# RobotLocomotion/pytorch-dense-correspondence

Hardware: AMD Instinct MI355X
Metric: training images/sec, 640x480 D=3 ResNet34-8s (higher is better)
Workload: dtype f32 (f16x3 products)

## Files before the change

pytorch-dense-correspondence_amd/csrc/conv_kernels.hip:

```cpp
#include "conv_shared.h"
#include "dcn_tuning.h"

namespace {

using namespace dcnconv;

template <int WM, int TM, int TN, int BK, bool TR>
__device__ __forceinline__ void gemm_segment(const GemmConv& p, float* lds, int tile, int k0, int k1, int nk, float* slot) {
    using G = GemmGeo<WM, TM, TN, BK>;
    constexpr int BM = G::BM, BN = G::BN, LDK = G::LDK, KQ = G::KQ, ROWS = G::ROWS, PA = G::PA, PB = G::PB,
                  kStage = G::kStage;
    const int tid = threadIdx.x, lane = tid & 63, wv = tid >> 6;
    const int wm_ = WM == 2 ? (wv >> 1) : 0, wn_ = WM == 2 ? (wv & 1) : wv;
    const int mt = fdiv(tile, p.div_nt), nt = tile - mt * p.ntiles;
    const int m0 = mt * BM, n0 = nt * BN;

    const int kq = tid % KQ, r0 = tid / KQ;
    int by[PA], bx[PA], pixbase[PA];
#pragma unroll
    for (int j = 0; j < PA; ++j) {
        const int m = m0 + r0 + ROWS * j;
        const int mm = m < p.M ? m : 0;
        const int img = fdiv(mm, p.div_hw), rem = mm - img * p.div_hw.d;
        const int y = fdiv(rem, p.div_w), x = rem - y * p.div_w.d;
// ... 412 lines not shown
            store_tile(cur ^ 1);
            mfma_steps(0);
#pragma unroll
            for (int i = 0; i < 16; ++i) {
                __builtin_amdgcn_sched_group_barrier(0x008, 1, 0);
                __builtin_amdgcn_sched_group_barrier(0x306, 3, 0);
            }
            __syncthreads();
            load_tile(m_begin + (st + 2 < nsteps ? st + 2 : nsteps - 1) * WK);
            read_frags(cur ^ 1, 0, 0);
            mfma_steps(1);
#pragma unroll
            for (int i = 0; i < 16; ++i) {
                __builtin_amdgcn_sched_group_barrier(0x008, 1, 0);
                __builtin_amdgcn_sched_group_barrier(0x126, 6, 0);
            }
        }
    }
    float* out = p.slab + (int64_t)split * p.cout * p.K;
    const int kc = j0 + wn_ * 64 + 2 * fi;
    if (kc < p.K) {
#pragma unroll
        for (int tm = 0; tm < 2; ++tm) {
#pragma unroll
            for (int r = 0; r < 16; ++r) {
                const int n = n0 + wm_ * 64 + 2 * ((r & 3) + 8 * (r >> 2) + 4 * fh) + tm;
                if (n < p.cout)
                    *reinterpret_cast<float2*>(out + (int64_t)n * p.K + kc) = make_float2(acc[tm][0][r], acc[tm][1][r]);
            }
        }
    }
}

__global__ void __launch_bounds__(256)
wgrad_reduce_kernel(const float* __restrict__ slab, float* __restrict__ dw, int64_t n4, int splits) {
    const int64_t i = (int64_t)blockIdx.x * 256 + threadIdx.x;
    if (i >= n4) return;
    const float4* src = reinterpret_cast<const float4*>(slab) + i;
    float4 a = src[0];
    int s = 1;
    for (; s + 4 <= splits; s += 4) {
        const float4 b0 = src[(int64_t)s * n4], b1 = src[(int64_t)(s + 1) * n4], b2 = src[(int64_t)(s + 2) * n4],
                     b3 = src[(int64_t)(s + 3) * n4];
        a.x += b0.x; a.y += b0.y; a.z += b0.z; a.w += b0.w;
        a.x += b1.x; a.y += b1.y; a.z += b1.z; a.w += b1.w;
        a.x += b2.x; a.y += b2.y; a.z += b2.z; a.w += b2.w;
        a.x += b3.x; a.y += b3.y; a.z += b3.z; a.w += b3.w;
    }
    for (; s < splits; ++s) {
        const float4 b = src[(int64_t)s * n4];
        a.x += b.x; a.y += b.y; a.z += b.z; a.w += b.w;
    }
    reinterpret_cast<float4*>(dw)[i] = a;
}

__global__ void __launch_bounds__(256)
wgrad_reduce_wide_kernel(const float* __restrict__ slab, float* __restrict__ dw, int64_t n4, int splits) {
    __shared__ float4 part[16][16];
    const int c = threadIdx.x & 15, sl = threadIdx.x >> 4;
    const int64_t i = (int64_t)blockIdx.x * 16 + c;
    float4 a = make_float4(0.f, 0.f, 0.f, 0.f);
    if (i < n4) {
        const float4* src = reinterpret_cast<const float4*>(slab) + i;
        int s = sl;
        for (; s + 48 < splits; s += 64) {
            const float4 b0 = src[(int64_t)s * n4], b1 = src[(int64_t)(s + 16) * n4], b2 = src[(int64_t)(s + 32) * n4],
                         b3 = src[(int64_t)(s + 48) * n4];
            a.x += b0.x; a.y += b0.y; a.z += b0.z; a.w += b0.w;
            a.x += b1.x; a.y += b1.y; a.z += b1.z; a.w += b1.w;
            a.x += b2.x; a.y += b2.y; a.z += b2.z; a.w += b2.w;
            a.x += b3.x; a.y += b3.y; a.z += b3.z; a.w += b3.w;
        }
        for (; s < splits; s += 16) {
            const float4 b = src[(int64_t)s * n4];
            a.x += b.x; a.y += b.y; a.z += b.z; a.w += b.w;
        }
    }
    part[sl][c] = a;
    __syncthreads();
    if (sl == 0 && i < n4) {
#pragma unroll
        for (int k = 1; k < 16; ++k) {
            const float4 b = part[k][c];
            a.x += b.x; a.y += b.y; a.z += b.z; a.w += b.w;
        }
        reinterpret_cast<float4*>(dw)[i] = a;
    }
}

__global__ void __launch_bounds__(256)
transpose_weight_kernel(const float* __restrict__ w, float* __restrict__ wt, int cout, int taps, int cin, int ldn) {
    __shared__ float tile[32][33];
    const int tap = blockIdx.z;
    const int c0 = blockIdx.x * 32, n0 = blockIdx.y * 32;
    const int tx = threadIdx.x & 31, ty = threadIdx.x >> 5;
    for (int i = ty; i < 32; i += 8) {
        const int n = n0 + i, c = c0 + tx;
        tile[i][tx] = (n < cout && c < cin) ? w[((int64_t)n * taps + tap) * cin + c] : 0.f;
    }
    __syncthreads();
    for (int i = ty; i < 32; i += 8) {
        const int c = c0 + i, n = n0 + tx;
        if (c < cin && n < ldn) wt[((int64_t)c * taps + tap) * ldn + n] = tile[tx][i];
    }
}

int wgrad_splits(const dcn_conv_desc* c, int* rows_per_split) {
    const int M = c->n * c->hout * c->wout, K = c->kh * c->kw * c->cin;
    const bool narrow = c->cout <= 64;
    const int tiles = dcn::ceil_div(c->cout, narrow ? 64 : 128) * dcn::ceil_div(K, narrow ? 256 : 128);
    int splits = dcn::ceil_div(2048, tiles);
    const int max_by_rows = (M / (8 * WK)) > 1 ? (M / (8 * WK)) : 1;
    if (splits > max_by_rows) splits = max_by_rows;
    const int cap = narrow ? 256 : 64;
    if (splits > cap) splits = cap;
    if (splits < 1) splits = 1;
    int rps = dcn::ceil_div(dcn::ceil_div(M, splits), WK) * WK;
    splits = dcn::ceil_div(M, rps);
    *rows_per_split = rps;
    return splits;
}

bool valid_desc(const dcn_conv_desc* c) {
    return c && c->n > 0 && c->hin > 0 && c->win > 0 && c->cin > 0 && (c->cin % 4) == 0 && c->hout > 0 && c->wout > 0 &&
           c->cout > 0 && c->kh > 0 && c->kw > 0 && c->stride > 0 && c->dil > 0 && c->pad >= 0 && c->ldc >= c->cout;
}

}

namespace dcnconv {
void launch_wgrad_reduce(const float* slabs, float* dw, int64_t n4, int splits, hipStream_t st) {
    if (splits >= 32) {
        hipLaunchKernelGGL(wgrad_reduce_wide_kernel, dim3((unsigned)dcn::ceil_div64(n4, 16)), dim3(256), 0, st, slabs, dw, n4, splits);
        return;
    }
    hipLaunchKernelGGL(wgrad_reduce_kernel, dim3((unsigned)dcn::ceil_div64(n4, 256)), dim3(256), 0, st, slabs, dw, n4,
                       splits);
}
}

extern "C" int dcn_conv_num_mtiles(const dcn_conv_desc* c) {
    if (!valid_desc(c)) return DCN_E_INVALID;
    return gemm_shape(c->n * c->hout * c->wout, c->cout, c->kh * c->kw * c->cin, c->group_rows).mtiles;
}

extern "C" size_t dcn_conv_gemm_workspace(const dcn_conv_desc* c, int dgrad) {
    if (!valid_desc(c)) return 0;
    if (dgrad) return gemm_shape(c->n * c->hin * c->win, c->cin, c->kh * c->kw * c->ldc).ws_bytes;
    return gemm_shape(c->n * c->hout * c->wout, c->cout, c->kh * c->kw * c->cin, c->group_rows).ws_bytes;
}

extern "C" int dcn_conv_forward(const dcn_conv_desc* c, const float* in, const float* w, const float* bias, float* out,
                                float* bn_partial, void* workspace, void* stream) {
    if (!valid_desc(c) || !in || !w || !out) return DCN_E_INVALID;
    GemmConv p;
    p.src = in; p.wm = w; p.bias = bias; p.add = nullptr; p.dst = out; p.bn_partial = bn_partial; p.out_absmax = nullptr;
    p.hs = c->hin; p.ws = c->win; p.cs = c->cin; p.hd = c->hout; p.wd = c->wout; p.cd = c->cout;
    p.kh = c->kh; p.kw = c->kw; p.stride = c->stride; p.pad = c->pad; p.dil = c->dil; p.ldc = c->ldc;
    p.M = c->n * c->hout * c->wout; p.K = c->kh * c->kw * c->cin; p.transposed = 0; p.relu = 0;
    return launch_gemm(p, workspace, (hipStream_t)stream, c->group_rows);
}

extern "C" int dcn_conv_dgrad(const dcn_conv_desc* c, const float* dout, const float* wt, const float* add, float* din,
                              void* workspace, void* stream) {
    if (!valid_desc(c) || !dout || !wt || !din || (c->ldc % 4) != 0) return DCN_E_INVALID;
    GemmConv p;
    p.src = dout; p.wm = wt; p.bias = nullptr; p.add = add; p.dst = din; p.bn_partial = nullptr; p.out_absmax = nullptr;
    p.hs = c->hout; p.ws = c->wout; p.cs = c->ldc;
    p.hd = c->hin; p.wd = c->win; p.cd = c->cin;
    p.kh = c->kh; p.kw = c->kw; p.stride = c->stride; p.pad = c->pad; p.dil = c->dil; p.ldc = c->cin;
// ... 42 lines not shown
```

pytorch-dense-correspondence_amd/csrc/conv_shared.h:

```cpp
#pragma once
#include <cstdlib>

#include "dcn_common.h"

namespace dcnconv {

typedef float f32x16 __attribute__((ext_vector_type(16)));

constexpr int NT = 256;

struct FastDiv {
    uint32_t mul, shr;
    int d;
};
inline FastDiv make_fastdiv(int d) {
    FastDiv f;
    f.d = d;
    uint32_t s = 0;
    while ((1u << s) < (uint32_t)d) ++s;
    f.shr = s;
    f.mul = (uint32_t)((((uint64_t)1 << 32) * (((uint64_t)1 << s) - (uint64_t)d)) / (uint64_t)d) + 1u;
    return f;
}
__device__ __forceinline__ int fdiv(int n, const FastDiv& f) { return (int)((__umulhi((uint32_t)n, f.mul) + (uint32_t)n) >> f.shr); }
// ... 220 lines not shown
            }
        }
    }
    if (p.bn_partial) {
#pragma unroll
        for (int tn = 0; tn < TN16; ++tn) {
            csum[tn] += __shfl_xor(csum[tn], 16, 64);
            csq[tn] += __shfl_xor(csq[tn], 16, 64);
            cmax[tn] = fmaxf(cmax[tn], __shfl_xor(cmax[tn], 16, 64));
            csum[tn] += __shfl_xor(csum[tn], 32, 64);
            csq[tn] += __shfl_xor(csq[tn], 32, 64);
            cmax[tn] = fmaxf(cmax[tn], __shfl_xor(cmax[tn], 32, 64));
            if (fq == 0) {
                const int cl = col0 + tn * 16 + fc;
                red[(wm * 3 + 0) * BN + cl] = csum[tn];
                red[(wm * 3 + 1) * BN + cl] = csq[tn];
                red[(wm * 3 + 2) * BN + cl] = cmax[tn];
            }
        }
        __syncthreads();
        if (tid < BN && n0 + tid < p.cd) {
            const float s = red[0 * BN + tid] + red[3 * BN + tid];
            const float q = red[1 * BN + tid] + red[4 * BN + tid];
            const float mx = fmaxf(red[2 * BN + tid], red[5 * BN + tid]);
            p.bn_partial[((int64_t)mt * 3 + 0) * p.cd + n0 + tid] = s;
            p.bn_partial[((int64_t)mt * 3 + 1) * p.cd + n0 + tid] = q;
            p.bn_partial[((int64_t)mt * 3 + 2) * p.cd + n0 + tid] = mx;
        }
    }
}

void launch_wgrad_reduce(const float* slabs, float* dw, int64_t n4, int splits, hipStream_t st);

}
```

pytorch-dense-correspondence_amd/csrc/dcn_tuning.h:

```cpp
#pragma once

namespace dcn {

struct Tuning {
    int conv_mode = -1;
    int conv_mode_invalid = 0;
    int backward_overlap = 1;
    int gemm_tile_m = 0;
    int gemm_sk = -1;
    double gemm_sk_min_gain = 20.0;
    int gemm_uni = 1;
    int stem8 = 1;
    int gemm_sk_inline = 1;
    int bn_bwd_fused = 0;
    int defer_residual_add = 1;
    int wgrad_splits = 0;
    int wgrad_tile = 0;
    int wgrad_deep = 4;
    int gemm_hl = 1;
    int hl_min_k = 128;
    int gemm_hl_rows = 0;
    int gemm_hlx = 1;
    int gemm_hlx_kg = 0;
    int gemm_hlx_splits = 0;
    int gemm_hlx_narrow = 1;
    double hlx_cost1 = 1.32, hlx_cost2 = 1.42, hlx_split_cost = 14.0;
    int hl_setprio = 1;
    int hlx_stagger = 1;
    int hlx_counters = 1;
    int wgrad_hl_min_m = 0;
    int wgrad_hl = 1;
    int wgrad_hlr = 1;
    int wgrad_hlr_min_m = 0;
    int wgrad_hlr_pairs = 1;
    int hl_producers = 1;
    int hl_only_mid = 1;
    int stem_pool_fused = 1;
    int bn_reduce_wide = 32;
    int wsplit_overlap = 1;
    int bn_nt = 0;
    int bn_reverse = 0;
    int wgrad_roles = 1;
};

const Tuning& tuning();

}
```

pytorch-dense-correspondence_amd/csrc/dcn_tuning.hip:

```cpp
#include <atomic>
#include <cstdio>
#include <cstdlib>
#include <cstring>
#include <mutex>

#include "dcn_common.h"
#include "dcn_tuning.h"

namespace dcn {
namespace {

Tuning g_tuning;
std::once_flag g_once;
std::mutex g_mu;

void read_env(Tuning& t) {
    t = Tuning();
    if (const char* m = getenv("DCN_CONV_MODE")) {
        if (!strcmp(m, "fp32")) t.conv_mode = DCN_CONV_FP32;
        else if (!strcmp(m, "f16x3")) t.conv_mode = DCN_CONV_F16X3;
        else t.conv_mode_invalid = 1;
    }
    if (const char* e = getenv("DCN_BACKWARD_OVERLAP")) t.backward_overlap = atoi(e) != 0;
    if (const char* e = getenv("DCN_GEMM_TILE_M")) t.gemm_tile_m = atoi(e);
// ... 8 lines not shown
    if (const char* e = getenv("DCN_WGRAD_ROLES")) t.wgrad_roles = atoi(e);
    if (const char* e = getenv("DCN_WGRAD_TILE")) t.wgrad_tile = atoi(e);
    if (const char* e = getenv("DCN_WGRAD_SPLITS")) t.wgrad_splits = atoi(e);
    if (const char* e = getenv("DCN_GEMM_HL")) t.gemm_hl = atoi(e);
    if (const char* e = getenv("DCN_GEMM_HL_ROWS")) t.gemm_hl_rows = atoi(e);
    if (const char* e = getenv("DCN_HL_MIN_K")) { const int v = atoi(e); if (v >= 32) t.hl_min_k = v; }
    if (const char* e = getenv("DCN_GEMM_HLX")) {
        int a = 0, b = 0;
        if (strchr(e, ',')) {
            if (sscanf(e, "%d,%d", &a, &b) == 2) {
                t.gemm_hlx = 1;
                t.gemm_hlx_kg = (a == 1 || a == 2) ? a : 0;
                t.gemm_hlx_splits = b > 0 ? b : 0;
            }
        } else {
            t.gemm_hlx = atoi(e) != 0;
        }
    }
    if (const char* e = getenv("DCN_GEMM_HLX_NARROW")) t.gemm_hlx_narrow = atoi(e) != 0;
    if (const char* e = getenv("DCN_HLX_COST")) {
        double a = 0, b = 0, c = 0;
        if (sscanf(e, "%lf,%lf,%lf", &a, &b, &c) == 3 && a > 0 && b > 0 && c >= 0) { t.hlx_cost1 = a; t.hlx_cost2 = b; t.hlx_split_cost = c; }
    }
    if (const char* e = getenv("DCN_HL_ONLY_MID")) t.hl_only_mid = atoi(e);
    if (const char* e = getenv("DCN_STEM_POOL_FUSED")) t.stem_pool_fused = atoi(e);
    if (const char* e = getenv("DCN_WGRAD_HL")) t.wgrad_hl = atoi(e);
    if (const char* e = getenv("DCN_HL_SETPRIO")) t.hl_setprio = atoi(e) != 0;
    if (const char* e = getenv("DCN_HLX_STAGGER")) { const int v = atoi(e); t.hlx_stagger = (v >= 0 && v <= 2) ? v : 1; }
    if (const char* e = getenv("DCN_HLX_COUNTERS")) t.hlx_counters = atoi(e) != 0;
    if (const char* e = getenv("DCN_WGRAD_HL_MIN_M")) t.wgrad_hl_min_m = atoi(e);
    if (const char* e = getenv("DCN_WGRAD_HLR")) t.wgrad_hlr = atoi(e);
    if (const char* e = getenv("DCN_WGRAD_HLR_MIN_M")) t.wgrad_hlr_min_m = atoi(e);
    if (const char* e = getenv("DCN_WGRAD_HLR_PAIRS")) t.wgrad_hlr_pairs = atoi(e);
    if (const char* e = getenv("DCN_HL_PRODUCERS")) t.hl_producers = atoi(e) != 0;
    if (const char* e = getenv("DCN_BN_REVERSE")) t.bn_reverse = atoi(e);
    if (const char* e = getenv("DCN_BN_NT")) t.bn_nt = atoi(e);
    if (const char* e = getenv("DCN_WSPLIT_OVERLAP")) t.wsplit_overlap = atoi(e) != 0;
    if (const char* e = getenv("DCN_BN_REDUCE_WIDE")) t.bn_reduce_wide = atoi(e);
}

}

const Tuning& tuning() {
    std::call_once(g_once, [] { read_env(g_tuning); });
    return g_tuning;
}

}

extern "C" void dcn_reload_env(void) {
    (void)dcn::tuning();
    std::lock_guard<std::mutex> lock(dcn::g_mu);
    dcn::read_env(dcn::g_tuning);
}
```

pytorch-dense-correspondence_amd/csrc/wgrad_hl_kernels.hip:

```cpp
#include <algorithm>
#include <type_traits>

#include "conv_shared.h"
#include "dcn_tuning.h"
#include "f16_split.h"

namespace {

using namespace dcnconv;
using namespace dcnsplit;

typedef __attribute__((address_space(3))) void* whl_lds_ptr;
typedef short s4v __attribute__((ext_vector_type(4)));

constexpr int kOob = (int)0x80000000;
constexpr int kStage = 65536;
constexpr int WPX = 32;

__device__ __forceinline__ void glds16(__amdgpu_buffer_rsrc_t rs, void* lds_dst, int voffset, int soffset) {
    __builtin_amdgcn_raw_ptr_buffer_load_lds(rs, (whl_lds_ptr)lds_dst, 16, voffset, soffset, 0, 0);
}
__device__ __forceinline__ s4v lds_tr4(const unsigned char* p) {
    return __builtin_amdgcn_ds_read_tr16_b64_v4i16((__attribute__((address_space(3))) s4v*)p);
}

struct WgradHl {
    const void* xh;
    const void* dh;
    float* slab;
    const float* x_absmax;
    const float* d_absmax;
    unsigned x_bytes, d_bytes;
    int hin, win, cin, cout, kh, kw, pad, dil, ldo, M, K, splits, stages_per_split, ntiles_n, ntiles_k, cpt, setprio;
    FastDiv div_hw, div_w, div_cpt, div_kw;
};

__global__ void __launch_bounds__(512, 1)
conv_wgrad_hl_kernel(WgradHl p) {
    __shared__ __attribute__((aligned(16))) unsigned char lds[2 * kStage];
    const int tid = threadIdx.x, lane = tid & 63;
    const int wv = __builtin_amdgcn_readfirstlane(tid >> 6);
    const int grp = wv >> 2, wn = wv & 3;
    const int tiles = p.ntiles_n * p.ntiles_k;
    const int bid = xcd_remap(blockIdx.x, tiles * p.splits);
    const int split = bid / tiles, tile = bid - split * tiles;
    const int tn_ = tile / p.ntiles_k, tk_ = tile - tn_ * p.ntiles_k;
    const int n0 = tn_ * 256, kc0 = tk_ * 256;
    const int nstages = (p.M + WPX - 1) / WPX;
    const int s_begin = split * p.stages_per_split;
    const int s_end = min(nstages, s_begin + p.stages_per_split);
    const int m_end = min(p.M, s_end * WPX);
    const __amdgpu_buffer_rsrc_t rs_x = __builtin_amdgcn_make_buffer_rsrc(const_cast<void*>(p.xh), 0, (int)p.x_bytes, 0x00020000);
    const __amdgpu_buffer_rsrc_t rs_d = __builtin_amdgcn_make_buffer_rsrc(const_cast<void*>(p.dh), 0, (int)p.d_bytes, 0x00020000);

    const int lp = lane >> 5, p16 = lane & 31;
    const int ldo4 = p.ldo * 4, cin4 = p.cin * 4;
    int kp[2];
    int cA[2][2], cB[2][2];
    int tdy[2][2], tdx[2][2];
#pragma unroll
    for (int e = 0; e < 2; ++e) {
        kp[e] = 4 * wv + 2 * e + lp;
        const int key = (kp[e] & 3) | (((kp[e] >> 3) & 1) << 2);
        const int unit = (p16 >> 1) ^ key;
        const int slot = unit >> 1;
        const int lc = slot >> 1, pl = slot & 1, q16 = 2 * (unit & 1) + (p16 & 1);
// ... 135 lines not shown
        else if (ph == 1) DCN_WAIT_VMCNT(0);
        DCN_WAIT_LGKMCNT0();
        bar();
        mfma_quadrant(qi, qj);
        bar();
    };
    using T = std::true_type;
    using F = std::false_type;
    if (s_begin < s_end) {
        issue_half(0, 0);
        issue_half(0, 1);
        issue_half(0, 2);
        issue_half(0, 3);
        advance();
        __builtin_amdgcn_sched_barrier(0);
        DCN_WAIT_VMCNT(4);
        bar();
        if (grp == 1) bar();
        int buf = 0;
        for (int s = s_begin; s + 1 < s_end; ++s) {
            phase(T{}, buf, 0);
            phase(T{}, buf, 1);
            phase(T{}, buf, 2);
            phase(T{}, buf, 3);
            buf ^= 1;
        }
        phase(F{}, buf, 0);
        phase(F{}, buf, 1);
        phase(F{}, buf, 2);
        phase(F{}, buf, 3);
        if (grp == 0) bar();
    }
    const float inv = 1.f / ((p.d_absmax ? pow2_scale(*p.d_absmax) : 1.f) * (p.x_absmax ? pow2_scale(*p.x_absmax) : 1.f));
    float* out = p.slab + (int64_t)split * p.cout * p.K;
    const int fc = lane & 15, fq4 = 4 * (lane >> 4);
#pragma unroll
    for (int tb = 0; tb < 8; ++tb)
#pragma unroll
        for (int cb = 0; cb < 4; ++cb) {
            const int kc = kc0 + wn * 64 + cb * 16 + fc;
#pragma unroll
            for (int r = 0; r < 4; ++r) {
                const int n = n0 + grp * 128 + tb * 16 + fq4 + r;
                if (n < p.cout && kc < p.K) out[(int64_t)n * p.K + kc] = acc[tb][cb][r] * inv;
            }
        }
}

bool wgrad_hl_supported(const dcn_conv_desc* c) {
    if (!c || c->n < 1 || c->hin < 1 || c->win < 32 || c->cin < 32 || c->cout < 32 || c->kh < 1 || c->kw < 1) return false;
    if (c->stride != 1 || c->hin != c->hout || c->win != c->wout || c->ldc != c->cout) return false;
    if ((c->cin % 32) != 0 || (c->cout % 32) != 0) return false;
    const int64_t xb = (int64_t)c->n * c->hin * c->win * c->cin * 4, db = (int64_t)c->n * c->hout * c->wout * c->ldc * 4;
    return xb <= ((int64_t)1 << 31) - 1 && db <= ((int64_t)1 << 31) - 1;
}

int wgrad_hl_splits(const dcn_conv_desc* c, int* stages_per_split) {
    const int M = c->n * c->hout * c->wout, K = c->kh * c->kw * c->cin;
    const int tiles = dcn::ceil_div(c->cout, 256) * dcn::ceil_div(K, 256);
    const int nstages = dcn::ceil_div(M, WPX);
    int best = 1;
    double best_score = -1.0;
    const int hi = std::min(nstages, std::max(1, 2 * 256 / tiles + 1));
    for (int s = 1; s <= hi; ++s) {
        const int sps = dcn::ceil_div(nstages, s), real = dcn::ceil_div(nstages, sps);
        const int wgs = real * tiles;
        const double eff = (double)wgs / (double)(dcn::ceil_div(wgs, 256) * 256);
        const double score = eff - 0.002 * real - (wgs < 256 ? 0.5 * (1.0 - wgs / 256.0) : 0.0) - (wgs > 256 ? 0.15 : 0.0);
        if (score > best_score) { best_score = score; best = s; }
    }
    if (const int v = dcn::tuning().wgrad_splits) { if (v >= 1 && v <= nstages) best = v; }
    const int sps = dcn::ceil_div(nstages, best);
    *stages_per_split = sps;
    return dcn::ceil_div(nstages, sps);
}


constexpr int RW_WP = 34;
constexpr int RW_DY_BYTES = 32 * 256;

template <int CB> struct RwGeom {
    static constexpr int kPitch = 256 * CB;
    static constexpr int kXInstr = (3 * RW_WP * kPitch + 8191) / 8192;
    static constexpr int kXBytes = kXInstr * 8192;
    static constexpr int kStageBytes = RW_DY_BYTES + kXBytes;
};

struct WgradHlr {
    const void* xh;
    const void* dh;
    float* slab;
    const float* x_absmax;
    const float* d_absmax;
    unsigned x_bytes, d_bytes;
    int hin, win, cin, cout, ldo, K, nstages, segs, splits, stages_per_split, ntiles_n, ntiles_c;
    FastDiv div_segs, div_h;
};

template <int CB>
__global__ void __launch_bounds__(512, 1)
conv_wgrad_hlr_kernel(WgradHlr p) {
    using G = RwGeom<CB>;
    constexpr int E = G::kXInstr, PITCH = G::kPitch;
    __shared__ __attribute__((aligned(16))) unsigned char lds[2 * G::kStageBytes];
    const int tid = threadIdx.x, lane = tid & 63;
    const int wv = __builtin_amdgcn_readfirstlane(tid >> 6);
    const int nh = wv & 1, cq = wv >> 1;
    const int tiles = p.ntiles_n * p.ntiles_c;
    const int bid = xcd_remap(blockIdx.x, tiles * p.splits);
    const int split = bid / tiles, tile = bid - split * tiles;
    const int tn_ = tile / p.ntiles_c, tc_ = tile - tn_ * p.ntiles_c;
    const int n0 = tn_ * 64, c0 = tc_ * 64 * CB;
    const int s_begin = split * p.stages_per_split;
    const int s_end = min(p.nstages, s_begin + p.stages_per_split);
    const __amdgpu_buffer_rsrc_t rs_x = __builtin_amdgcn_make_buffer_rsrc(const_cast<void*>(p.xh), 0, (int)p.x_bytes, 0x00020000);
    const __amdgpu_buffer_rsrc_t rs_d = __builtin_amdgcn_make_buffer_rsrc(const_cast<void*>(p.dh), 0, (int)p.d_bytes, 0x00020000);
    auto key_of = [](int pixel) { return (pixel & 3) | (((pixel >> 3) & 1) << 2); };

    auto unit_src = [](int u, int ps) { return (u >> 2) * 128 + ((u >> 1) & 1) * 64 + (u & 1) * 32 + (ps & 1) * 16; };
    const int dpix = 4 * wv + (lane >> 4);
    const int dsrc = (n0 / 32) * 128 + unit_src(((lane & 15) >> 1) ^ key_of(dpix), lane & 15);
    int xinfo[E];
#pragma unroll
    for (int e = 0; e < E; ++e) {
        const int byte = (wv + 8 * e) * 1024 + lane * 16;
        const int row = byte / PITCH, ps = (byte - row * PITCH) >> 4;
        const int r = row / RW_WP, q = row - r * RW_WP;
        xinfo[e] = unit_src((ps >> 1) ^ key_of(q), ps) | (q << 16) | ((row < 3 * RW_WP ? r + 1 : 0) << 24);
// ... 83 lines not shown
            if constexpr (CB == 1) DCN_WAIT_VMCNT(5); else DCN_WAIT_VMCNT(8);
        } else {
            __builtin_amdgcn_sched_barrier(0);
            DCN_WAIT_VMCNT(0);
        }
        __builtin_amdgcn_sched_barrier(0);
        __builtin_amdgcn_s_barrier();
        __builtin_amdgcn_sched_barrier(0);
        va = abase + buf * G::kStageBytes;
        DCN_OPAQUE_INT(va);
#pragma unroll
        for (int sft = 0; sft < 3; ++sft)
#pragma unroll
            for (int h = 0; h < 2; ++h) {
                vb[sft][h] = bbase[sft][h] + buf * G::kStageBytes;
                DCN_OPAQUE_INT(vb[sft][h]);
            }
        read_a();
#pragma unroll
        for (int tap = 0; tap < AH; ++tap) read_b(tap, tap);
#pragma unroll
        for (int tap = 0; tap < 9; ++tap) {
            if (tap + AH < 9) read_b(tap + AH, (tap + AH) % (AH + 1));
            __builtin_amdgcn_sched_barrier(0);
            mfma_tap(tap, tap % (AH + 1));
            __builtin_amdgcn_sched_barrier(0);
        }
        __builtin_amdgcn_sched_barrier(0);
        DCN_WAIT_LGKMCNT0();
        __builtin_amdgcn_s_barrier();
        __builtin_amdgcn_sched_barrier(0);
    }
    const float inv = 1.f / ((p.d_absmax ? pow2_scale(*p.d_absmax) : 1.f) * (p.x_absmax ? pow2_scale(*p.x_absmax) : 1.f));
    float* out = p.slab + (int64_t)split * p.cout * p.K;
    const int fc = lane & 15, fq4 = 4 * (lane >> 4);
#pragma unroll
    for (int i = 0; i < 2; ++i)
#pragma unroll
        for (int tap = 0; tap < 9; ++tap)
#pragma unroll
            for (int c = 0; c < CB; ++c) {
                const int kc = tap * p.cin + c0 + (CB * cq + c) * 16 + fc;
#pragma unroll
                for (int r = 0; r < 4; ++r) {
                    const int n = n0 + (2 * nh + i) * 16 + fq4 + r;
                    out[(int64_t)n * p.K + kc] = acc[i][tap][c][r] * inv;
                }
            }
}


constexpr int RP_DY_BYTES = 2 * 32 * 256;
constexpr int RP_XINSTR = 5;
constexpr int RP_STAGE = RP_DY_BYTES + RP_XINSTR * 8192;

__global__ void __launch_bounds__(512, 1)
conv_wgrad_hlrp_kernel(WgradHlr p) {
    constexpr int E = RP_XINSTR, PITCH = 256;
    __shared__ __attribute__((aligned(16))) unsigned char lds[2 * RP_STAGE];
    const int tid = threadIdx.x, lane = tid & 63;
    const int wv = __builtin_amdgcn_readfirstlane(tid >> 6);
    const int grp = wv >> 2, cq = wv & 3;
    const int tiles = p.ntiles_n * p.ntiles_c;
    const int bid = xcd_remap(blockIdx.x, tiles * p.splits);
    const int split = bid / tiles, tile = bid - split * tiles;
    const int tn_ = tile / p.ntiles_c, tc_ = tile - tn_ * p.ntiles_c;
// ... 118 lines not shown
        }
        __builtin_amdgcn_sched_barrier(0);
        DCN_WAIT_LGKMCNT0();
        __builtin_amdgcn_s_barrier();
        __builtin_amdgcn_sched_barrier(0);
    }
    float4* xch = reinterpret_cast<float4*>(lds);
#pragma unroll
    for (int half = 0; half < 2; ++half) {
        if (grp == 1) {
#pragma unroll
            for (int i = 0; i < 2; ++i)
#pragma unroll
                for (int tap = 0; tap < 9; ++tap) {
                    const f32x4_t v = acc[2 * half + i][tap];
                    xch[(cq * 18 + i * 9 + tap) * 64 + lane] = make_float4(v[0], v[1], v[2], v[3]);
                }
        }
        __syncthreads();
        if (grp == 0) {
#pragma unroll
            for (int i = 0; i < 2; ++i)
#pragma unroll
                for (int tap = 0; tap < 9; ++tap) {
                    const float4 v = xch[(cq * 18 + i * 9 + tap) * 64 + lane];
                    acc[2 * half + i][tap][0] += v.x; acc[2 * half + i][tap][1] += v.y;
                    acc[2 * half + i][tap][2] += v.z; acc[2 * half + i][tap][3] += v.w;
                }
        }
        __syncthreads();
    }
    if (grp != 0) return;
    const float inv = 1.f / ((p.d_absmax ? pow2_scale(*p.d_absmax) : 1.f) * (p.x_absmax ? pow2_scale(*p.x_absmax) : 1.f));
    float* out = p.slab + (int64_t)split * p.cout * p.K;
    const int fc = lane & 15, fq4 = 4 * (lane >> 4);
#pragma unroll
    for (int i = 0; i < 4; ++i)
#pragma unroll
        for (int tap = 0; tap < 9; ++tap) {
            const int kc = tap * p.cin + c0 + cq * 16 + fc;
#pragma unroll
            for (int r = 0; r < 4; ++r) out[(int64_t)(n0 + i * 16 + fq4 + r) * p.K + kc] = acc[i][tap][r] * inv;
        }
}

bool wgrad_hlr_supported(const dcn_conv_desc* c) {
    if (!c || c->n < 1 || c->hin < 1 || c->win < 1 || c->hout < 1 || c->wout < 1 || c->kh != 3 || c->kw != 3 || c->dil != 1 ||
        c->pad != 1) return false;
    if (c->stride != 1 || c->hin != c->hout || c->win != c->wout || c->ldc != c->cout) return false;
    if (c->cin < 64 || c->cout < 64 || (c->cin % 64) != 0 || (c->cout % 64) != 0) return false;
    const int64_t xb = (int64_t)c->n * c->hin * c->win * c->cin * 4, db = (int64_t)c->n * c->hout * c->wout * c->ldc * 4;
    return xb <= ((int64_t)1 << 31) - 1 && db <= ((int64_t)1 << 31) - 1;
}
bool hlr_pairs() { return dcn::tuning().wgrad_hlr_pairs != 0; }
int wgrad_hlr_stages(const dcn_conv_desc* c, bool pairs) {
    return c->n * (pairs ? dcn::ceil_div(c->hout, 2) : c->hout) * dcn::ceil_div(c->wout, 32);
}
int wgrad_hlr_splits(const dcn_conv_desc* c, int* stages_per_split, bool pairs) {
    const int nstages = wgrad_hlr_stages(c, pairs), tiles = (c->cout / 64) * (c->cin / 64);
    int s = std::max(1, std::min(std::max(256 / tiles, 1), nstages / 2));
    if (const int v = dcn::tuning().wgrad_splits) { if (v >= 1 && v <= nstages) s = v; }
    const int sps = dcn::ceil_div(nstages, s);
    *stages_per_split = sps;
    return dcn::ceil_div(nstages, sps);
}
bool use_hlr(const dcn_conv_desc* c) {
    const int v = dcn::tuning().wgrad_hlr;
    if (v == 0 || !wgrad_hlr_supported(c)) return false;
    if (v == 2) return true;
    if ((c->cout % 256) == 0) return false;
    if (dcn::tuning().wgrad_hlr_min_m > 0) return (int64_t)c->n * c->hout * c->wout >= dcn::tuning().wgrad_hlr_min_m;
    return (int64_t)c->n * c->hout * dcn::ceil_div(c->wout, 32) * (c->cout / 64) * (c->cin / 64) >= 2048;
}
int launch_wgrad_hlr(const dcn_conv_desc* c, const void* x_hl, const float* x_absmax, const void* dout_hl,
                     const float* dout_absmax, float* dw, void* slabs, hipStream_t st) {
    WgradHlr p;
    p.xh = x_hl; p.dh = dout_hl; p.x_absmax = x_absmax; p.d_absmax = dout_absmax;
    p.x_bytes = (unsigned)((int64_t)c->n * c->hin * c->win * c->cin * 4);
    p.d_bytes = (unsigned)((int64_t)c->n * c->hout * c->wout * c->ldc * 4);
    p.hin = c->hin; p.win = c->win; p.cin = c->cin; p.cout = c->cout; p.ldo = c->ldc; p.K = 9 * c->cin;
    p.segs = dcn::ceil_div(c->wout, 32); p.nstages = wgrad_hlr_stages(c, hlr_pairs());
    p.splits = wgrad_hlr_splits(c, &p.stages_per_split, hlr_pairs());
    p.ntiles_n = c->cout / 64; p.ntiles_c = c->cin / 64;
    p.div_segs = make_fastdiv(p.segs); p.div_h = make_fastdiv(hlr_pairs() ? dcn::ceil_div(c->hin, 2) : c->hin);
    p.slab = p.splits == 1 ? dw : (float*)slabs;
    if (hlr_pairs()) hipLaunchKernelGGL(conv_wgrad_hlrp_kernel, dim3(p.ntiles_n * p.ntiles_c * p.splits), dim3(512), 0, st, p);
    else hipLaunchKernelGGL(conv_wgrad_hlr_kernel<1>, dim3(p.ntiles_n * p.ntiles_c * p.splits), dim3(512), 0, st, p);
    if (p.splits > 1) launch_wgrad_reduce((const float*)slabs, dw, (int64_t)c->cout * p.K / 4, p.splits, st);
    return dcn::check_launch();
}
}

extern "C" int dcn_conv_wgrad_hl_eligible(const dcn_conv_desc* c) {
    if (dcn::tuning().wgrad_hl == 0) return 0;
    if (use_hlr(c)) return 1;
    if (!wgrad_hl_supported(c)) return 0;
    if (dcn::tuning().wgrad_hl == 2) return 1;
    const int64_t min_m = dcn::tuning().wgrad_hl_min_m > 0 ? dcn::tuning().wgrad_hl_min_m : 4096;
    return ((c->cout % 256) == 0 && c->kh * c->kw * c->cin >= std::min(1024, dcn::tuning().hl_min_k) &&
            (int64_t)c->n * c->hout * c->wout >= min_m) ? 1 : 0;
}

extern "C" int dcn_conv_wgrad_hl_kind(const dcn_conv_desc* c) { return use_hlr(c) ? 2 : (wgrad_hl_supported(c) ? 1 : 0); }

extern "C" size_t dcn_conv_wgrad_workspace_hl(const dcn_conv_desc* c) {
    size_t bytes = 0;
    int sps;
    if (wgrad_hlr_supported(c))
        bytes = (size_t)std::max(wgrad_hlr_splits(c, &sps, true), wgrad_hlr_splits(c, &sps, false)) * c->cout * 9 * c->cin * sizeof(float);
    if (wgrad_hl_supported(c))
        bytes = std::max(bytes, (size_t)wgrad_hl_splits(c, &sps) * c->cout * c->kh * c->kw * c->cin * sizeof(float));
    return bytes;
}

extern "C" int dcn_conv_wgrad_hl(const dcn_conv_desc* c, const void* x_hl, const float* x_absmax, const void* dout_hl,
                                 const float* dout_absmax, float* dw, void* slabs, void* stream) {
    if (!x_hl || !dout_hl || !dw || !slabs) return DCN_E_INVALID;
    if (use_hlr(c)) return launch_wgrad_hlr(c, x_hl, x_absmax, dout_hl, dout_absmax, dw, slabs, (hipStream_t)stream);
    if (!wgrad_hl_supported(c)) return DCN_E_UNSUPPORTED;
    WgradHl p;
    p.xh = x_hl; p.dh = dout_hl; p.x_absmax = x_absmax; p.d_absmax = dout_absmax;
    p.x_bytes = (unsigned)((int64_t)c->n * c->hin * c->win * c->cin * 4);
    p.d_bytes = (unsigned)((int64_t)c->n * c->hout * c->wout * c->ldc * 4);
    p.hin = c->hin; p.win = c->win; p.cin = c->cin; p.cout = c->cout; p.kh = c->kh; p.kw = c->kw; p.pad = c->pad; p.dil = c->dil;
    p.ldo = c->ldc; p.M = c->n * c->hout * c->wout; p.K = c->kh * c->kw * c->cin; p.cpt = c->cin / 32;
    p.splits = wgrad_hl_splits(c, &p.stages_per_split);
    p.setprio = dcn::tuning().hl_setprio;
    p.ntiles_n = dcn::ceil_div(c->cout, 256); p.ntiles_k = dcn::ceil_div(p.K, 256);
    p.div_hw = make_fastdiv(c->hout * c->wout); p.div_w = make_fastdiv(c->wout);
    p.div_cpt = make_fastdiv(p.cpt); p.div_kw = make_fastdiv(c->kw);
    p.slab = p.splits == 1 ? dw : (float*)slabs;
    hipStream_t st = (hipStream_t)stream;
    hipLaunchKernelGGL(conv_wgrad_hl_kernel, dim3(p.ntiles_n * p.ntiles_k * p.splits), dim3(512), 0, st, p);
    if (p.splits > 1) launch_wgrad_reduce((const float*)slabs, dw, (int64_t)c->cout * p.K / 4, p.splits, st);
    return dcn::check_launch();
}
```

Before: 465.4.

## Store split-K wgrad partials in fragment order and scatter during reduction

When weight-gradient GEMMs are split across multiple slabs, each wave now writes its accumulator fragments as contiguous float4 per lane in MFMA fragment order, instead of scattering them into the row-major dW layout. A new reduce kernel sums the slabs in that layout and maps each fragment back to its (cout, k) position when writing dW. This makes the partial-slab writes and reads fully coalesced, at the cost of strided scalar stores in the final reduce and extra index arithmetic. Workspace sizing for the non-HLR path is changed to cover whole padded tiles.

```diff
diff --git a/pytorch-dense-correspondence_amd/csrc/conv_kernels.hip b/pytorch-dense-correspondence_amd/csrc/conv_kernels.hip
--- a/pytorch-dense-correspondence_amd/csrc/conv_kernels.hip
+++ b/pytorch-dense-correspondence_amd/csrc/conv_kernels.hip
@@ -468,11 +468,7 @@
     }
 }
 
-__global__ void __launch_bounds__(256)
-wgrad_reduce_kernel(const float* __restrict__ slab, float* __restrict__ dw, int64_t n4, int splits) {
-    const int64_t i = (int64_t)blockIdx.x * 256 + threadIdx.x;
-    if (i >= n4) return;
-    const float4* src = reinterpret_cast<const float4*>(slab) + i;
+__device__ __forceinline__ float4 sum_slabs_in_order(const float4* __restrict__ src, int64_t n4, int splits) {
     float4 a = src[0];
     int s = 1;
     for (; s + 4 <= splits; s += 4) {
@@ -487,7 +483,31 @@
         const float4 b = src[(int64_t)s * n4];
         a.x += b.x; a.y += b.y; a.z += b.z; a.w += b.w;
     }
-    reinterpret_cast<float4*>(dw)[i] = a;
+    return a;
+}
+__device__ __forceinline__ float4 sum_slabs_of_lane(const float4* __restrict__ src, int64_t n4, int splits, int sl) {
+    float4 a = make_float4(0.f, 0.f, 0.f, 0.f);
+    int s = sl;
+    for (; s + 48 < splits; s += 64) {
+        const float4 b0 = src[(int64_t)s * n4], b1 = src[(int64_t)(s + 16) * n4], b2 = src[(int64_t)(s + 32) * n4],
+                     b3 = src[(int64_t)(s + 48) * n4];
+        a.x += b0.x; a.y += b0.y; a.z += b0.z; a.w += b0.w;
+        a.x += b1.x; a.y += b1.y; a.z += b1.z; a.w += b1.w;
+        a.x += b2.x; a.y += b2.y; a.z += b2.z; a.w += b2.w;
+        a.x += b3.x; a.y += b3.y; a.z += b3.z; a.w += b3.w;
+    }
+    for (; s < splits; s += 16) {
+        const float4 b = src[(int64_t)s * n4];
+        a.x += b.x; a.y += b.y; a.z += b.z; a.w += b.w;
+    }
+    return a;
+}
+
+__global__ void __launch_bounds__(256)
+wgrad_reduce_kernel(const float* __restrict__ slab, float* __restrict__ dw, int64_t n4, int splits) {
+    const int64_t i = (int64_t)blockIdx.x * 256 + threadIdx.x;
+    if (i >= n4) return;
+    reinterpret_cast<float4*>(dw)[i] = sum_slabs_in_order(reinterpret_cast<const float4*>(slab) + i, n4, splits);
 }
 
 __global__ void __launch_bounds__(256)
@@ -496,22 +516,7 @@
     const int c = threadIdx.x & 15, sl = threadIdx.x >> 4;
     const int64_t i = (int64_t)blockIdx.x * 16 + c;
     float4 a = make_float4(0.f, 0.f, 0.f, 0.f);
-    if (i < n4) {
-        const float4* src = reinterpret_cast<const float4*>(slab) + i;
-        int s = sl;
-        for (; s + 48 < splits; s += 64) {
-            const float4 b0 = src[(int64_t)s * n4], b1 = src[(int64_t)(s + 16) * n4], b2 = src[(int64_t)(s + 32) * n4],
-                         b3 = src[(int64_t)(s + 48) * n4];
-            a.x += b0.x; a.y += b0.y; a.z += b0.z; a.w += b0.w;
-            a.x += b1.x; a.y += b1.y; a.z += b1.z; a.w += b1.w;
-            a.x += b2.x; a.y += b2.y; a.z += b2.z; a.w += b2.w;
-            a.x += b3.x; a.y += b3.y; a.z += b3.z; a.w += b3.w;
-        }
-        for (; s < splits; s += 16) {
-            const float4 b = src[(int64_t)s * n4];
-            a.x += b.x; a.y += b.y; a.z += b.z; a.w += b.w;
-        }
-    }
+    if (i < n4) a = sum_slabs_of_lane(reinterpret_cast<const float4*>(slab) + i, n4, splits, sl);
     part[sl][c] = a;
     __syncthreads();
     if (sl == 0 && i < n4) {
@@ -521,6 +526,69 @@
             a.x += b.x; a.y += b.y; a.z += b.z; a.w += b.w;
         }
         reinterpret_cast<float4*>(dw)[i] = a;
+    }
+}
+
+template <int KIND>
+__device__ __forceinline__ void wgrad_frag_pos(int64_t q, const WgradFragMap& m, int& n, int& kc) {
+    constexpr int T4 = KIND == WGRAD_FRAG_TILE ? 256 * 256 / 4 : 64 * 576 / 4;
+    constexpr int FR = KIND == WGRAD_FRAG_TILE ? 32 : KIND == WGRAD_FRAG_ROWPAIR ? 36 : 18;
+    const int tile = (int)(q / T4), rem = (int)(q - (int64_t)tile * T4);
+    const int wv = rem / (FR * 64), f = (rem >> 6) - wv * FR, lane = rem & 63;
+    const int ta = tile / m.ntiles_minor, tb = tile - ta * m.ntiles_minor;
+    const int fc = lane & 15, fq4 = 4 * (lane >> 4);
+    if (KIND == WGRAD_FRAG_TILE) {
+        n = ta * 256 + (wv >> 2) * 128 + (f >> 2) * 16 + fq4;
+        kc = tb * 256 + (wv & 3) * 64 + (f & 3) * 16 + fc;
+    } else if (KIND == WGRAD_FRAG_ROWPAIR) {
+        const int i = f / 9, tap = f - 9 * i;
+        n = ta * 64 + i * 16 + fq4;
+        kc = tap * m.cin + tb * 64 + wv * 16 + fc;
+    } else {
+        const int i = f / 9, tap = f - 9 * i;
+        n = ta * 64 + (2 * (wv & 1) + i) * 16 + fq4;
+        kc = tap * m.cin + tb * 64 + (wv >> 1) * 16 + fc;
+    }
+}
+__device__ __forceinline__ void wgrad_frag_store(float* __restrict__ dw, const WgradFragMap& m, int n, int kc, float4 a) {
+    if (kc >= m.K) return;
+    float* o = dw + (int64_t)n * m.K + kc;
+    if (n < m.cout) o[0] = a.x;
+    if (n + 1 < m.cout) o[m.K] = a.y;
+    if (n + 2 < m.cout) o[2 * (int64_t)m.K] = a.z;
+    if (n + 3 < m.cout) o[3 * (int64_t)m.K] = a.w;
+}
+
+template <int KIND>
+__global__ void __launch_bounds__(256)
+wgrad_reduce_frag_kernel(const float* __restrict__ slab, float* __restrict__ dw, int64_t n4, int splits, WgradFragMap m) {
+    const int64_t q = (int64_t)blockIdx.x * 256 + threadIdx.x;
+    if (q >= n4) return;
+    const float4 a = sum_slabs_in_order(reinterpret_cast<const float4*>(slab) + q, n4, splits);
+    int n, kc;
+    wgrad_frag_pos<KIND>(q, m, n, kc);
+    wgrad_frag_store(dw, m, n, kc, a);
+}
+
+template <int KIND>
+__global__ void __launch_bounds__(256)
+wgrad_reduce_frag_wide_kernel(const float* __restrict__ slab, float* __restrict__ dw, int64_t n4, int splits, WgradFragMap m) {
+    __shared__ float4 part[16][16];
+    const int c = threadIdx.x & 15, sl = threadIdx.x >> 4;
+    const int64_t q = (int64_t)blockIdx.x * 16 + c;
+    float4 a = make_float4(0.f, 0.f, 0.f, 0.f);
+    if (q < n4) a = sum_slabs_of_lane(reinterpret_cast<const float4*>(slab) + q, n4, splits, sl);
+    part[sl][c] = a;
+    __syncthreads();
+    if (sl == 0 && q < n4) {
+#pragma unroll
+        for (int k = 1; k < 16; ++k) {
+            const float4 b = part[k][c];
+            a.x += b.x; a.y += b.y; a.z += b.z; a.w += b.w;
+        }
+        int n, kc;
+        wgrad_frag_pos<KIND>(q, m, n, kc);
+        wgrad_frag_store(dw, m, n, kc, a);
     }
 }
 
@@ -572,6 +640,22 @@
     }
     hipLaunchKernelGGL(wgrad_reduce_kernel, dim3((unsigned)dcn::ceil_div64(n4, 256)), dim3(256), 0, st, slabs, dw, n4,
                        splits);
+}
+
+template <int KIND>
+static void launch_wgrad_reduce_frag_kind(const float* slabs, float* dw, int64_t n4, int splits, const WgradFragMap& m, hipStream_t st) {
+    if (splits >= 32)
+        hipLaunchKernelGGL(wgrad_reduce_frag_wide_kernel<KIND>, dim3((unsigned)dcn::ceil_div64(n4, 16)), dim3(256), 0, st, slabs, dw,
+                           n4, splits, m);
+    else
+        hipLaunchKernelGGL(wgrad_reduce_frag_kernel<KIND>, dim3((unsigned)dcn::ceil_div64(n4, 256)), dim3(256), 0, st, slabs, dw, n4,
+                           splits, m);
+}
+void launch_wgrad_reduce_frag(const float* slabs, float* dw, int tiles, int splits, const WgradFragMap& m, hipStream_t st) {
+    const int64_t n4 = (int64_t)tiles * (wgrad_frag_tile_elems(m.kind) / 4);
+    if (m.kind == WGRAD_FRAG_TILE) launch_wgrad_reduce_frag_kind<WGRAD_FRAG_TILE>(slabs, dw, n4, splits, m, st);
+    else if (m.kind == WGRAD_FRAG_ROWPAIR) launch_wgrad_reduce_frag_kind<WGRAD_FRAG_ROWPAIR>(slabs, dw, n4, splits, m, st);
+    else launch_wgrad_reduce_frag_kind<WGRAD_FRAG_ROW>(slabs, dw, n4, splits, m, st);
 }
 }
 
diff --git a/pytorch-dense-correspondence_amd/csrc/conv_shared.h b/pytorch-dense-correspondence_amd/csrc/conv_shared.h
--- a/pytorch-dense-correspondence_amd/csrc/conv_shared.h
+++ b/pytorch-dense-correspondence_amd/csrc/conv_shared.h
@@ -276,4 +276,14 @@
 
 void launch_wgrad_reduce(const float* slabs, float* dw, int64_t n4, int splits, hipStream_t st);
 
-}
+enum { WGRAD_FRAG_TILE = 0,
+       WGRAD_FRAG_ROWPAIR = 1,
+       WGRAD_FRAG_ROW = 2 };
+struct WgradFragMap {
+    int kind, cout, K, cin;
+    int ntiles_minor;
+};
+constexpr int wgrad_frag_tile_elems(int kind) { return kind == WGRAD_FRAG_TILE ? 256 * 256 : 64 * 576; }
+void launch_wgrad_reduce_frag(const float* slabs, float* dw, int tiles, int splits, const WgradFragMap& m, hipStream_t st);
+
+}
diff --git a/pytorch-dense-correspondence_amd/csrc/dcn_tuning.h b/pytorch-dense-correspondence_amd/csrc/dcn_tuning.h
--- a/pytorch-dense-correspondence_amd/csrc/dcn_tuning.h
+++ b/pytorch-dense-correspondence_amd/csrc/dcn_tuning.h
@@ -33,6 +33,7 @@
     int wgrad_hlr = 1;
     int wgrad_hlr_min_m = 0;
     int wgrad_hlr_pairs = 1;
+    int wgrad_slab_frag = 1;
     int hl_producers = 1;
     int hl_only_mid = 1;
     int stem_pool_fused = 1;
diff --git a/pytorch-dense-correspondence_amd/csrc/dcn_tuning.hip b/pytorch-dense-correspondence_amd/csrc/dcn_tuning.hip
--- a/pytorch-dense-correspondence_amd/csrc/dcn_tuning.hip
+++ b/pytorch-dense-correspondence_amd/csrc/dcn_tuning.hip
@@ -64,6 +64,7 @@
     if (const char* e = getenv("DCN_WGRAD_HLR")) t.wgrad_hlr = atoi(e);
     if (const char* e = getenv("DCN_WGRAD_HLR_MIN_M")) t.wgrad_hlr_min_m = atoi(e);
     if (const char* e = getenv("DCN_WGRAD_HLR_PAIRS")) t.wgrad_hlr_pairs = atoi(e);
+    if (const char* e = getenv("DCN_WGRAD_SLAB_FRAG")) t.wgrad_slab_frag = atoi(e) != 0;
     if (const char* e = getenv("DCN_HL_PRODUCERS")) t.hl_producers = atoi(e) != 0;
     if (const char* e = getenv("DCN_BN_REVERSE")) t.bn_reverse = atoi(e);
     if (const char* e = getenv("DCN_BN_NT")) t.bn_nt = atoi(e);
diff --git a/pytorch-dense-correspondence_amd/csrc/wgrad_hl_kernels.hip b/pytorch-dense-correspondence_amd/csrc/wgrad_hl_kernels.hip
--- a/pytorch-dense-correspondence_amd/csrc/wgrad_hl_kernels.hip
+++ b/pytorch-dense-correspondence_amd/csrc/wgrad_hl_kernels.hip
@@ -22,6 +22,14 @@
 }
 __device__ __forceinline__ s4v lds_tr4(const unsigned char* p) {
     return __builtin_amdgcn_ds_read_tr16_b64_v4i16((__attribute__((address_space(3))) s4v*)p);
+}
+
+template <int NWV, int NFR>
+__device__ __forceinline__ float4* frag_slot(float* slab, int split, int tiles, int tile, int wv, int lane) {
+    return reinterpret_cast<float4*>(slab) + (((int64_t)split * tiles + tile) * NWV + wv) * (NFR * 64) + lane;
+}
+__device__ __forceinline__ void park(float4* slot, int f, const f32x4_t& v, float inv) {
+    slot[f * 64] = make_float4(v[0] * inv, v[1] * inv, v[2] * inv, v[3] * inv);
 }
 
 struct WgradHl {
@@ -31,7 +39,7 @@
     const float* x_absmax;
     const float* d_absmax;
     unsigned x_bytes, d_bytes;
-    int hin, win, cin, cout, kh, kw, pad, dil, ldo, M, K, splits, stages_per_split, ntiles_n, ntiles_k, cpt, setprio;
+    int hin, win, cin, cout, kh, kw, pad, dil, ldo, M, K, splits, stages_per_split, ntiles_n, ntiles_k, cpt, setprio, frag;
     FastDiv div_hw, div_w, div_cpt, div_kw;
 };
 
@@ -233,6 +241,14 @@
         if (grp == 0) bar();
     }
     const float inv = 1.f / ((p.d_absmax ? pow2_scale(*p.d_absmax) : 1.f) * (p.x_absmax ? pow2_scale(*p.x_absmax) : 1.f));
+    if (p.frag) {
+        float4* slot = frag_slot<8, 32>(p.slab, split, tiles, tile, wv, lane);
+#pragma unroll
+        for (int tb = 0; tb < 8; ++tb)
+#pragma unroll
+            for (int cb = 0; cb < 4; ++cb) park(slot, tb * 4 + cb, acc[tb][cb], inv);
+        return;
+    }
     float* out = p.slab + (int64_t)split * p.cout * p.K;
     const int fc = lane & 15, fq4 = 4 * (lane >> 4);
 #pragma unroll
@@ -294,7 +310,7 @@
     const float* x_absmax;
     const float* d_absmax;
     unsigned x_bytes, d_bytes;
-    int hin, win, cin, cout, ldo, K, nstages, segs, splits, stages_per_split, ntiles_n, ntiles_c;
+    int hin, win, cin, cout, ldo, K, nstages, segs, splits, stages_per_split, ntiles_n, ntiles_c, frag;
     FastDiv div_segs, div_h;
 };
 
@@ -444,6 +460,16 @@
         __builtin_amdgcn_sched_barrier(0);
     }
     const float inv = 1.f / ((p.d_absmax ? pow2_scale(*p.d_absmax) : 1.f) * (p.x_absmax ? pow2_scale(*p.x_absmax) : 1.f));
+    if constexpr (CB == 1) {
+        if (p.frag) {
+            float4* slot = frag_slot<8, 18>(p.slab, split, tiles, tile, wv, lane);
+#pragma unroll
+            for (int i = 0; i < 2; ++i)
+#pragma unroll
+                for (int tap = 0; tap < 9; ++tap) park(slot, i * 9 + tap, acc[i][tap][0], inv);
+            return;
+        }
+    }
     float* out = p.slab + (int64_t)split * p.cout * p.K;
     const int fc = lane & 15, fq4 = 4 * (lane >> 4);
 #pragma unroll
@@ -628,6 +654,14 @@
     }
     if (grp != 0) return;
     const float inv = 1.f / ((p.d_absmax ? pow2_scale(*p.d_absmax) : 1.f) * (p.x_absmax ? pow2_scale(*p.x_absmax) : 1.f));
+    if (p.frag) {
+        float4* slot = frag_slot<4, 36>(p.slab, split, tiles, tile, cq, lane);
+#pragma unroll
+        for (int i = 0; i < 4; ++i)
+#pragma unroll
+            for (int tap = 0; tap < 9; ++tap) park(slot, i * 9 + tap, acc[i][tap], inv);
+        return;
+    }
     float* out = p.slab + (int64_t)split * p.cout * p.K;
     const int fc = lane & 15, fq4 = 4 * (lane >> 4);
 #pragma unroll
@@ -680,9 +714,15 @@
     p.ntiles_n = c->cout / 64; p.ntiles_c = c->cin / 64;
     p.div_segs = make_fastdiv(p.segs); p.div_h = make_fastdiv(hlr_pairs() ? dcn::ceil_div(c->hin, 2) : c->hin);
     p.slab = p.splits == 1 ? dw : (float*)slabs;
+    p.frag = (p.splits > 1 && dcn::tuning().wgrad_slab_frag) ? 1 : 0;
     if (hlr_pairs()) hipLaunchKernelGGL(conv_wgrad_hlrp_kernel, dim3(p.ntiles_n * p.ntiles_c * p.splits), dim3(512), 0, st, p);
     else hipLaunchKernelGGL(conv_wgrad_hlr_kernel<1>, dim3(p.ntiles_n * p.ntiles_c * p.splits), dim3(512), 0, st, p);
-    if (p.splits > 1) launch_wgrad_reduce((const float*)slabs, dw, (int64_t)c->cout * p.K / 4, p.splits, st);
+    if (p.frag) {
+        const WgradFragMap m = {hlr_pairs() ? WGRAD_FRAG_ROWPAIR : WGRAD_FRAG_ROW, c->cout, p.K, c->cin, p.ntiles_c};
+        launch_wgrad_reduce_frag((const float*)slabs, dw, p.ntiles_n * p.ntiles_c, p.splits, m, st);
+    } else if (p.splits > 1) {
+        launch_wgrad_reduce((const float*)slabs, dw, (int64_t)c->cout * p.K / 4, p.splits, st);
+    }
     return dcn::check_launch();
 }
 }
@@ -705,7 +745,8 @@
     if (wgrad_hlr_supported(c))
         bytes = (size_t)std::max(wgrad_hlr_splits(c, &sps, true), wgrad_hlr_splits(c, &sps, false)) * c->cout * 9 * c->cin * sizeof(float);
     if (wgrad_hl_supported(c))
-        bytes = std::max(bytes, (size_t)wgrad_hl_splits(c, &sps) * c->cout * c->kh * c->kw * c->cin * sizeof(float));
+        bytes = std::max(bytes, (size_t)wgrad_hl_splits(c, &sps) * dcn::ceil_div(c->cout, 256) * dcn::ceil_div(c->kh * c->kw * c->cin, 256) *
+                                    wgrad_frag_tile_elems(WGRAD_FRAG_TILE) * sizeof(float));
     return bytes;
 }
 
@@ -726,8 +767,14 @@
     p.div_hw = make_fastdiv(c->hout * c->wout); p.div_w = make_fastdiv(c->wout);
     p.div_cpt = make_fastdiv(p.cpt); p.div_kw = make_fastdiv(c->kw);
     p.slab = p.splits == 1 ? dw : (float*)slabs;
+    p.frag = (p.splits > 1 && dcn::tuning().wgrad_slab_frag) ? 1 : 0;
     hipStream_t st = (hipStream_t)stream;
     hipLaunchKernelGGL(conv_wgrad_hl_kernel, dim3(p.ntiles_n * p.ntiles_k * p.splits), dim3(512), 0, st, p);
-    if (p.splits > 1) launch_wgrad_reduce((const float*)slabs, dw, (int64_t)c->cout * p.K / 4, p.splits, st);
+    if (p.frag) {
+        const WgradFragMap m = {WGRAD_FRAG_TILE, c->cout, p.K, c->cin, p.ntiles_k};
+        launch_wgrad_reduce_frag((const float*)slabs, dw, p.ntiles_n * p.ntiles_k, p.splits, m, st);
+    } else if (p.splits > 1) {
+        launch_wgrad_reduce((const float*)slabs, dw, (int64_t)c->cout * p.K / 4, p.splits, st);
+    }
     return dcn::check_launch();
 }
```

Measured after the change: 465.2. About the same (-0.0%).
